# uricchio/2DSFS-scan

Measured on AMD Instinct MI355X. Metric: genomic windows/s (T2D+T1D+Fst) at 20 kb, n1=n2=50; HBM GB/s fraction, higher is better.
Workload: dtype f64

## Files before the change

### 2dsfs-scan_amd/csrc/sfs2d.hip

```cpp
#include <hip/hip_runtime.h>
#include <hip/hip_ext.h>

#include <algorithm>
#include <array>
#include <cmath>
#include <cstdint>
#include <cstdio>
#include <cstdlib>
#include <cstring>
#include <map>
#include <string>
#include <mutex>
#include <new>
#include <utility>
#include <vector>

#include "sfs2d.h"
#include "sfs2d_kernels.hpp"
#include "sfs2d_div.hpp"
#include "sfs2d_spec.hpp"
#include "sfs2d_proj.hpp"
#include "sfs2d_projscan.hpp"
#include "sfs2d_projnull.hpp"

// ... 170 lines not shown
  int tevery = 1;
  int tmask = 7;
  int64_t tseen = 0;
  hipEvent_t* tpend = nullptr;
  hipEvent_t kev[6] = {nullptr, nullptr, nullptr, nullptr, nullptr, nullptr};
  std::vector<unsigned long long> slot_base_h;
  uint32_t* d_slot_base = nullptr;
  sfs2d_plan* base = nullptr;
  std::vector<sfs2d_plan*> attached;
  uint32_t fst_m = 0;
  bool fst_win = false;
  bool fst_scan = false;
  bool fst_mask = true;
  bool gate = false;
  bool lean = false;
  int nfst = 0;
  std::vector<NullTask> ntask_h;
  DevBuf<NullTask> ntask;
  CallOut<sfs2d_window, 0> null_out;
  int variant[6] = {-1, -1, -1, -1, -1, -1};
  bool variant_set = false;
  CallOut<sfs2d_diversity> div_out;
  std::vector<SpecSel> spec_sel_h;
  DevBuf<SpecSel> spec_sel;
  CallOut<int64_t> spec_out;
  std::vector<ProjSel> proj_sel_h;
  DevBuf<ProjSel> proj_sel;
  CallOut<int64_t> proj_out;
  int64_t proj_roww = 0;
  int proj_e = 0;
// ... 86 lines not shown

bool free_slots(const sfs2d_plan* pl) { return pl->step > 0 || pl->regions; }

struct ScanW {
  bool p16, fused;
  int fst;
  bool cnt, gate, lean;
  using Fn = void (*)(SCAN_W_ARGS);
  static constexpr int N = 128;
  constexpr int index() const { return p16 | fused << 1 | fst << 2 | cnt << 4 | gate << 5 | lean << 6; }
  static constexpr ScanW at(int i) { return {bool(i & 1), bool(i & 2), (i >> 2) & 3, bool(i & 16), bool(i & 32), bool(i & 64)}; }
  constexpr bool legal() const { return fst < 2 ? !gate && !lean : cnt && (gate || !lean); }
  template <int I> static constexpr Fn kernel() { constexpr ScanW s = at(I); return k_scan_w<s.p16, s.fused, s.fst, s.cnt, s.gate, s.lean>; }
};

struct ScanGW {
  bool p16, fst, cnt, tri;
  using Fn = void (*)(SCAN_W_ARGS);
  static constexpr int N = 16;
  constexpr int index() const { return p16 | fst << 1 | cnt << 2 | tri << 3; }
  static constexpr ScanGW at(int i) { return {bool(i & 1), bool(i & 2), bool(i & 4), bool(i & 8)}; }
  constexpr bool legal() const { return cnt || !tri; }
  template <int I> static constexpr Fn kernel() { constexpr ScanGW s = at(I); return k_scan_gw<s.p16, s.fst, s.cnt, s.tri>; }
};

struct ScanG {
  bool p16, fst, cnt;
  using Fn = decltype(&k_scan_g<true, true, true>);
  static constexpr int N = 8;
  constexpr int index() const { return p16 | fst << 1 | cnt << 2; }
// ... 116 lines not shown
size_t static_lds(S s, size_t fallback) {
  hipFuncAttributes fa{};
  return hipFuncGetAttributes(&fa, (const void*)variants<S>[s.index()]) == hipSuccess ? fa.sharedSizeBytes : fallback;
}
template <class S>
int occupancy(S s, int block, size_t lds) {
  int occ = 0;
  return hipOccupancyMaxActiveBlocksPerMultiprocessor(&occ, variants<S>[s.index()], block, lds) == hipSuccess ? occ : 0;
}

ScanW scan_w_sel(const sfs2d_plan* pl) {
  const bool in_scan = pl->cnt && pl->fst_scan;
  const int fst = in_scan ? (pl->fst_mask ? 3 : 2) : prep_sums_fst(pl) ? 1 : 0;
  return {pl->p16, pl->fused, fst, pl->cnt, in_scan && (pl->gate || pl->lean), in_scan && pl->lean};
}
ScanGW scan_gw_sel(const sfs2d_plan* pl) { return {pl->p16, prep_sums_fst(pl), pl->cnt, pl->cnt && pl->K.ntri}; }
ScanG scan_g_sel(const sfs2d_plan* pl) { return {pl->p16, prep_sums_fst(pl), pl->cnt}; }
ScanExtra scan_extra_sel(const sfs2d_plan* pl) { return {pl->p16, pl->cnt}; }

ScanW occ_standin(ScanW s) { s.fst = s.fst >= 2 ? 2 : 1; s.cnt = true; return s; }
ScanGW occ_standin(ScanGW s) { s.fst = s.cnt = true; return s; }

constexpr ScanW SCAN_W_FIT = {true, true, 1, true, false, false};
constexpr ScanW scan_w_fst_fit(bool p16) { return {p16, true, 2, true, false, false}; }
constexpr Prep prep_lds_fit(bool fst) { return {true, true, true, true, false, fst, false}; }

void set_variant(sfs2d_plan* pl, int p16, int fused, int fst, int cnt, int gate, int tri) {
  const int v[6] = {p16, fused, fst, cnt, gate, tri};
  std::copy(v, v + 6, pl->variant);
  pl->variant_set = true;
}

int launch_scan(sfs2d_plan* pl, sfs2d_window* out) {
  const int per_chrom = pl->prm.bg_mode == SFS2D_BG_PER_CHROM ? 1 : 0;
  const int bp = pl->prm.window_mode == SFS2D_WINDOW_BP ? 1 : 0;
  const dim3 grid((unsigned)pl->chunks.size());
  int rc = 0;
  if (pl->gw) {
    const ScanGW s = scan_gw_sel(pl);
    const ScanGW::Fn k = variant(pl->ctx, s, "k_scan_gw", &rc);
    if (!k) return rc;
    set_variant(pl, s.p16, -1, s.fst, s.cnt, -1, s.tri);
    hipExtLaunchKernelGGL(k, grid, dim3(WAVE), pl->scan_lds,
                       CTX_STREAM(pl->ctx), pl->kev[4], pl->kev[5], 0, pl->K, scan_src(pl), pl->d_chunks, pl->d_slots, pl->d_tab, pl->d_lp, pl->d_head,
                       per_chrom, pl->ctx->d_lnx, pl->ctx->d_df, out, pl->d_err, bp, pl->d_repl, pl->d_bcount,
                       0, pl->d_leaves, pl->nleaves, pl->d_nodes, pl->nnodes, pl->nlevels, -1, pl->d_fsum, pl->d_fst,
                       pl->d_ctr, (int)(pl->runs & 1), pl->d_leafsum, pl->d_bg1d, 0, pl->d_gscr, pl->nscr);
  } else if (pl->G == WAVE) {
    const ScanW s = scan_w_sel(pl);
    const ScanW::Fn k = variant(pl->ctx, s, "k_scan_w", &rc);
    if (!k) return rc;
    set_variant(pl, s.p16, s.fused, s.fst, s.cnt, s.gate, -1);
    hipExtLaunchKernelGGL(k, grid, dim3(SBLOCK), pl->scan_lds,
                       CTX_STREAM(pl->ctx), pl->kev[4], pl->kev[5], 0, pl->K, scan_src(pl), pl->d_chunks, pl->d_slots, pl->d_tab, pl->d_lp, pl->d_head,
                       per_chrom, pl->ctx->d_lnx, pl->ctx->d_df, out, pl->d_err, bp, pl->d_repl, pl->d_bcount,
                       plan_par(pl), pl->d_leaves, pl->nleaves, pl->d_nodes, pl->nnodes, pl->nlevels,
                       pl->extra_rec >= 0 ? (int)pl->last_chrom : -1, pl->d_fsum, pl->d_fst, pl->d_ctr,
                       (int)(pl->runs & 1), pl->d_leafsum, pl->d_bg1d, pl->sliced ? 1 : 0, nullptr, 0);
  } else {
    const ScanG s = scan_g_sel(pl);
    const ScanG::Fn k = variant(pl->ctx, s, "k_scan_g", &rc);
    if (!k) return rc;
    set_variant(pl, s.p16, -1, s.fst, s.cnt, -1, -1);
    hipExtLaunchKernelGGL(k, grid, dim3(BLOCK), pl->scan_lds,
                       CTX_STREAM(pl->ctx), pl->kev[4], pl->kev[5], 0, pl->K, scan_src(pl), pl->d_chunks, pl->d_slots, pl->d_tab, pl->d_head, per_chrom,
// ... 518 lines not shown
  K->ws = (unsigned)prm->window;
  div_magic(K->ws, &K->wmag, &K->wsh1, &K->wsh2);
  K->nchrom = nchrom;
  K->fst_e = 40;
  K->fst_scale = std::ldexp(1.0, K->fst_e);
  return 0;
}

struct Knobs {
  const char* seg = std::getenv("SFS2D_SEG");
  const char* lnl = std::getenv("SFS2D_LNL");
  const char* gw = std::getenv("SFS2D_GW");
  const char* fused = std::getenv("SFS2D_FUSED");
  const char* fst_scan = std::getenv("SFS2D_FST_SCAN");
  const char* lean = std::getenv("SFS2D_LEAN");
  const char* slots_once = std::getenv("SFS2D_SLOTS_ONCE");
  const char* wgs = std::getenv("SFS2D_WGS");
  const char* gwwin = std::getenv("SFS2D_GWWIN");
  const char* pools = std::getenv("SFS2D_POOLS");
  const char* tile = std::getenv("SFS2D_TILE");
  const char* jnt = std::getenv("SFS2D_JNT");
};

struct RegionList {
  const int32_t* chrom;
  const uint32_t *first, *last;
  int64_t n;
};

static int plan_create(sfs2d_ctx* ctx, const sfs2d_data* data, const sfs2d_params* prm, int force_sliced, int64_t step,
// ... 222 lines not shown
  const bool small = pl->do_bg && pl->G == WAVE;
  const double wpw = (double)pl->nslots / (2.0 * ctx->ncu * (SBLOCK / WAVE));
  pl->sliced = small && wpw < 4.0;
  if (env.fused) pl->sliced = small && env.fused[0] == '0';
  if (force_sliced >= 0) pl->sliced = small && force_sliced == 1;
  pl->fused = small && !pl->sliced;
  pl->fst = (prm->flags & SFS2D_F_FST) != 0;
  pl->fst_scan = false;
  if (pl->fst && pl->cnt && pl->G == WAVE && !pl->gw) {
    pl->fst_scan = !(env.fst_scan && env.fst_scan[0] == '0');
    if (pl->fst_scan && pl->scan_lds + static_lds(scan_w_fst_fit(pl->p16), 160 * 1024) > 160 * 1024) pl->fst_scan = false;
  }
  pl->gate = pl->fst_scan && prm->fold && nc_ok;
  pl->lean = pl->gate && bp && K.n1p <= 31 && K.n2p <= 31;
  if (env.lean) pl->lean = pl->lean && env.lean[0] != '0';
  const PwTree pw = pw_plan(K.nb2 - 3);
  pl->fst_mask = data->low_nc;
  pl->fst_win = pl->sliced && bp && pl->fst && !pl->fst_scan;
  if (slide) pl->fst_win = pl->fst && !pl->fst_scan;
  pl->seg_index = bp && !slide && pl->cnt && pl->do_bg && !seg_prep && force_sliced < 0 && data->owned &&
                  !prep_sums_fst(pl);
  if (pl->seg_index) {
    if ((rc = data_pos_index(ctx, data))) { delete pl; return rc; }
    pl->do_seg = false;
  }
  pl->slots_once = pl->seg_index && pl->fst_scan;
  if (env.slots_once) pl->slots_once = pl->slots_once && env.slots_once[0] != '0';
  pl->nfst = pl->fst_win && !slide ? (int)std::min<int64_t>(1024, std::max<int64_t>(1, (pl->nslots + 7) / 8)) : 0;
  if (pl->scan_lds > 64 * 1024) {
    grant_lds<ScanW>(ctx, pl->scan_lds);
    grant_lds<ScanG>(ctx, pl->scan_lds);
  }
  if (pl->extra_lds > 64 * 1024) grant_lds<ScanExtra>(ctx, pl->extra_lds);

  if (pl->G == WAVE || pl->gw) {
    int occ = pl->gw ? occupancy(occ_standin(scan_gw_sel(pl)), WAVE, pl->scan_lds)
                     : occupancy(occ_standin(scan_w_sel(pl)), SBLOCK, pl->scan_lds);
    if (occ < 1) occ = 1;
    if (prm->scan_wgs_per_cu > 0 && (int)prm->scan_wgs_per_cu < occ) occ = (int)prm->scan_wgs_per_cu;
    int64_t cap = (int64_t)occ * ctx->ncu;
    if (pl->gw) pl->nscr = (int)cap;
    if (env.wgs) cap = std::max<int64_t>(1, std::atoll(env.wgs));
    const double S = (double)std::max<unsigned long long>(1, slot_base[nc] - slot_base[0]);
    const uint32_t NW = pl->gw ? 1u : (uint32_t)(SBLOCK / WAVE);
    int64_t gw_win = 64;
    if (env.gwwin) gw_win = std::max<int64_t>(1, std::atoll(env.gwwin));
    std::vector<double> order;
    for (int c = 0; c < nc; ++c) {
      const uint32_t ns = (uint32_t)(slot_base[c + 1] - slot_base[c]);
      if (!ns) continue;
      const uint32_t wmax = (ns + NW - 1) / NW;
      int64_t want = std::llround(cap * (ns / S));
// ... 248 lines not shown
  if (pl->base) return pl->step ? "slide" : pl->prm.window_mode == SFS2D_WINDOW_BP ? "bp" : "none";
  if (pl->step) return "slide";
  if (pl->seg_index) return "index";
  if (slots_only(pl)) return pl->seg_synth ? "synth" : "search";
  return pl->do_seg ? "prep" : "none";
}

int sfs2d_plan_slots_once(const sfs2d_plan* pl) { return !pl ? SFS2D_E_ARG : pl->slots_once ? 1 : 0; }

int sfs2d_plan_scan_variant(const sfs2d_plan* pl, int* p16, int* fused, int* fst, int* cnt, int* gate, int* tri) {
  if (!pl) return SFS2D_E_ARG;
  if (!pl->variant_set) return set_err(pl->ctx, SFS2D_E_ARG, "sfs2d_plan_scan_variant: the plan has launched no scan kernel yet");
  int* const o[6] = {p16, fused, fst, cnt, gate, tri};
  for (int i = 0; i < 6; ++i)
    if (o[i]) *o[i] = pl->variant[i];
  return 0;
}

int sfs2d_plan_set_timing(sfs2d_plan* pl, int max_runs) { return sfs2d_plan_set_timing_sampled(pl, max_runs, 1); }

int sfs2d_plan_set_timing_sampled(sfs2d_plan* pl, int max_runs, int every) {
  return sfs2d_plan_set_timing_kernels(pl, max_runs, every, 7);
}

int sfs2d_plan_set_timing_kernels(sfs2d_plan* pl, int max_runs, int every, int kernel_mask) {
  if (!pl || max_runs < 0 || every < 1 || (kernel_mask & ~7) || !kernel_mask) return SFS2D_E_ARG;
  pl->tevery = every;
  pl->tmask = kernel_mask;
  pl->tseen = 0;
  sfs2d_ctx* ctx = pl->ctx;
// ... 1323 lines not shown
```

### 2dsfs-scan_amd/csrc/sfs2d_kernels.hpp

```cpp
#pragma once

#include <type_traits>
#include <hip/hip_runtime.h>

#include <cmath>
#include <cstdint>

#include "sfs2d.h"

namespace sfs2dk {

constexpr int WAVE = 64;
constexpr int BLOCK = 256;
constexpr int SBLOCK = 512;
constexpr int BLOCK1 = 512;
constexpr int FBLOCK = 1024;
constexpr int KBLOCK = 512;
constexpr int LNX_N = 1 << 20;
constexpr int LNT = 512;
constexpr int LNF = 256;
__host__ __device__ inline int wl_rtn(int n1p, int n2p) { return 2 * (n1p > n2p ? n1p : n2p) + 2; }
constexpr int RCPN = 512;
#ifndef SFS2D_ABL
#define SFS2D_ABL 0
#endif
constexpr int REPL = 4;
constexpr int PW_MAX_LEAVES = 1024;
constexpr int LEAVES_PER_SLICE = 4;
constexpr int FIN_LDS_BINS = 12288;
constexpr int TRASH = WAVE;
constexpr int R1 = 4;
#ifndef SFS2D_GW_R1
#define SFS2D_GW_R1 1
#endif
constexpr int R1GW = SFS2D_GW_R1;

template <int RR>
__device__ __forceinline__ uint32_t take_replicas(uint32_t* p, uint32_t shift) {
  if (RR == 4) {
    uint4* q = reinterpret_cast<uint4*>(p);
    const uint4 v = *q;
    *q = make_uint4(0, 0, 0, 0);
    return (v.x >> shift) + (v.y >> shift) + (v.z >> shift) + (v.w >> shift);
  } else if (RR == 2) {
    uint2* q = reinterpret_cast<uint2*>(p);
    const uint2 v = *q;
    *q = make_uint2(0, 0);
    return (v.x >> shift) + (v.y >> shift);
  } else {
    const uint32_t v = *p;
    *p = 0u;
    return v >> shift;
  }
}
// ... 1355 lines not shown
    PL e;
    e.lp = LPl[k];
    if (k < nb2) {
      e.v = (double)u(k);
    } else if (k < t1b) {
      const int f = k - t1a;
      e.v = (double)u(h1a + f) + (f < n1p ? (double)u(h1a + n1 - f) : 0.0);
    } else {
      const int f = k - t1b, n2p = n2 / 2;
      e.v = (double)u(h1b + f) + (f < n2p ? (double)u(h1b + n2 - f) : 0.0);
    }
    return e;
  }
};

template <int G, bool P16, int S1, bool CNT, class Tab>
__device__ __forceinline__ WinOut eval_exact(const KParams& P, const uint32_t* __restrict__ bins, uint32_t b,
                                             uint32_t e, const Tab& T, const BgHead& hb,
                                             const double* __restrict__ lnx, uint32_t* H2, uint32_t* H1a,
                                             uint32_t* H1b, double* redd, unsigned long long* redu) {
  const int lane = threadIdx.x & (G - 1);
  const bool floatv = hb.flags & BGF_FLOATV;
  uint32_t c_var = 0, c2 = 0, c_last = 0, c1a = 0, c1b = 0;
  for (uint32_t i = b + lane; i < e; i += G) {
    const uint32_t w = snp_word<CNT>(P, bins, i);
    const uint32_t k2 = bin_k2(w), g1 = bin_g1(w), g2 = bin_g2(w);
    c_var += (w & B_VAR) ? 1u : 0u;
    c_last += (w & B_LAST) ? 1u : 0u;
    if (k2) { ++c2; h2_add<P16>(H2, k2); }
    if (g1) { ++c1a; atomicAdd(&H1a[g1 * S1], 1u); }
    if (g2) { ++c1b; atomicAdd(&H1b[g2 * S1], 1u); }
  }
  if (G == WAVE) __threadfence();
  group_sync<G>();
  const unsigned long long r0 = group_sum_u64<G>((unsigned long long)c2 | ((unsigned long long)c_last << 32), redu, 0);
  const unsigned long long r1 = group_sum_u64<G>((unsigned long long)c1a | ((unsigned long long)c1b << 32), redu, 1);
  const unsigned long long r2 = group_sum_u64<G>((unsigned long long)c_var, redu, 2);
  WinOut o;
  o.n2 = (uint32_t)r0;
  o.n2_all = o.n2 + (uint32_t)(r0 >> 32);
  o.n1a = (uint32_t)r1;
  o.n1b = (uint32_t)(r1 >> 32);
  o.snp_count = (uint32_t)r2;
  const double N2 = (double)o.n2, N1a = (double)o.n1a, N1b = (double)o.n1b;
// ... 27 lines not shown
        }
        __syncthreads();
      }
#pragma unroll
      for (int u = 0; u < U; ++u) {
        if (x2[u]) term(x2[u], (int)k2[u], N2, hb.B2, s2, q2);
        if (xa[u]) term(xa[u], P.t1a + (int)g1[u], N1a, hb.B1a, sa, qa);
        if (xb[u]) term(xb[u], P.t1b + (int)g2[u], N1b, hb.B1b, sb, qb);
      }
    }
  } else {
  for (uint32_t i = b + lane; i < e; i += G) {
    const uint32_t w = snp_word<CNT>(P, bins, i);
    const uint32_t k2 = bin_k2(w), g1 = bin_g1(w), g2 = bin_g2(w);
    if (k2) {
      const uint32_t x = h2_take<P16>(H2, k2);
      if (x) {
        const PL t = T.at(k2);
        s2 += (double)x * (lnx_of(lnx, x) - t.lp);
        q2 &= prop_ok(x, N2, t.v, hb.B2, floatv);
      }
    }
    if (g1) {
      const uint32_t x = atomicExch(&H1a[g1 * S1], 0u);
      if (x) {
        const PL t = T.at(P.t1a + g1);
        sa += (double)x * (lnx_of(lnx, x) - t.lp);
        qa &= prop_ok(x, N1a, t.v, hb.B1a, floatv);
      }
    }
    if (g2) {
// ... 666 lines not shown
}


__device__ __forceinline__ void lds_copy_d(double* dst, const double* __restrict__ src, int n) {
  constexpr int U = 8;
  for (int k0 = threadIdx.x; k0 < n; k0 += U * SBLOCK) {
    double v[U];
#pragma unroll
    for (int j = 0; j < U; ++j) v[j] = k0 + j * SBLOCK < n ? src[k0 + j * SBLOCK] : 0.0;
#pragma unroll
    for (int j = 0; j < U; ++j)
      if (k0 + j * SBLOCK < n) dst[k0 + j * SBLOCK] = v[j];
  }
}

template <bool P16, bool FUSED, int FST, bool CNT, bool GATE = false, bool LEAN = false>
__device__ __forceinline__ void scan_w_small(double* ldsd, uint32_t wgi, uint32_t nwg, SCAN_W_ARGS) {
  constexpr bool FSTIN = FST >= 2;
  constexpr bool FMASK = FST == 3;
  static_assert(!FSTIN || CNT, "Fst in the scan reads the counts");
  static_assert(!GATE || CNT, "the gate is a property of the counts the scan classifies");
  static_assert(!LEAN || (GATE && FSTIN), "the lean window loop is built for the gated Fst-in-scan plans");
  if (LEAN) mode_bp = 1;
  constexpr int DT = LNT;
  constexpr int R1U = R1;
  constexpr int NWV = SBLOCK / WAVE;
  constexpr int SB = 8;
  __shared__ BgHead sh_hb;
  __shared__ double sh_bd[NWV][3][SB];
  __shared__ uint32_t sh_bu[NWV][5][SB];
  __shared__ unsigned long long sh_bf[NWV][FST ? 2 : 1][SB];
  STAMP(10);
  BLK_STAMP(1, 0);
  const int tid = threadIdx.x;
  const int wv = __builtin_amdgcn_readfirstlane(tid >> 6);
  const int lane = tid & (WAVE - 1);
  const Chunk ch = chunks[wgi];
  const int bg = bg_per_chrom ? (int)ch.chrom : 0;

  double* LPl = ldsd;
  double* Dt = LPl + ((P.nt + 1) & ~1);
  double* Ft = Dt + DT;
  double2* RT = reinterpret_cast<double2*>(Ft + LNF);
  const int rtn = FSTIN ? P.rtn : 0;
  uint32_t* HB = reinterpret_cast<uint32_t*>(RT + rtn);
  const int h2w = P16 ? ((P.nb2 + 1) / 2 + 3) & ~3 : (P.nb2 + 3) & ~3;
  const int h1w = R1 * (P.n1p + 1), h1wb = R1 * (P.n2p + 1);
  const int per = (h2w + h1w + h1wb + 3) & ~3;
  uint32_t* W = HB + wv * per;
  uint32_t* H1a = W + h2w;
  uint32_t* H1b = H1a + h1w;
  const uint32_t rep = lane & (R1U - 1);

  auto bounds = [&](uint32_t s, uint2 sr, Win& w, bool live) {
    if (mode_bp) {
      w.has = live && sr.x != 0u;
      w.b = sr.x - 1u;
      w.e = sr.y;
    } else {
      w.has = live;
      w.b = ch.cb + (ch.wid_lo + (s - ch.slot_lo)) * P.ws;
      w.e = w.b + P.ws;
// ... 158 lines not shown
      }
    }
      if (mine && mode_bp && !FSTIN && !exact) {
        uint32_t z = 0u;
        asm volatile("" : "+v"(z));
        slots[Bs] = make_uint2(z, z);
      }
    MARK(31);
    for (unsigned long long m = __ballot(exact); m; m &= m - 1) {
      const int l = __builtin_ctzll(m);
      const uint32_t xs = __builtin_amdgcn_readlane(Bs, l), xb = __builtin_amdgcn_readlane(Bsb, l);
      const uint32_t xn = __builtin_amdgcn_readlane(Bnv, l) & 0xffffu;
      const uint32_t xe = xn != 0xffffu ? xb + xn : (mode_bp ? slots[xs].y : xb + P.ws);
      WinOut x;
      if (FUSED) {
        x = eval_exact<WAVE, P16, R1, CNT>(P, bins, xb, xe,
                                      TabFused{LPl, Rc, rs, P.nb2, P.n1, P.n2, P.n1p, P.h1a, P.h1b, P.t1a, P.t1b}, hb,
                                      lnx, W, H1a, H1b, nullptr, nullptr);
      } else {
        x = eval_exact<WAVE, P16, R1, CNT>(P, bins, xb, xe, TabLocal{tab + (size_t)bg * P.nt, LPl}, hb, lnx, W, H1a, H1b,
                                      nullptr, nullptr);
      }
      if (lane == 0) {
        write_rec(out + xs, ch.chrom, ch.wid_lo + (xs - ch.slot_lo), xb, xe, x, zflags);
        atomicAdd(err_word + 1, 1u);
      }
      group_sync<WAVE>();
    }
    jb = 0;
  };
#define SAT16(x) ((LEAN && P16) ? (x) : min((x), 0xffffu))
  auto put_u = [&](uint32_t slot, uint32_t b, uint32_t nsnp, uint32_t n2, uint32_t n1a, uint32_t n1b, uint32_t nvar,
                   uint32_t nlast) {
    sh_bu[wv][0][jb] = slot;
    sh_bu[wv][1][jb] = b;
// ... 90 lines not shown
        }
      }
    };
    auto pair = [&](uint32_t w0, uint32_t w1, int j, bool keep, const double2 (&fq)[4]) {
      const uint32_t ww[2] = {w0, w1};
      uint32_t rk[2], kk[2], ov[2], xs[2];
      bool in2[2];
#pragma unroll
      for (int q = 0; q < 2; ++q) {
        const uint32_t w = ww[q];
        uint32_t k2, gp;
        if (CNT) cls_k2g<GATE>(P, w, k2, gp);
        else { k2 = bin_k2(w); gp = bin_g1(w) | (bin_g2(w) << 16); }
        in2[q] = k2 != 0u;
        n2 += __popcll(__ballot(in2[q]));
        const uint32_t x = (CNT ? k2 : w) << 4;
        const uint32_t word = P16 ? (k2 >> 1) : k2;
        uint32_t one2 = 1u;
        if (P16) asm("v_lshlrev_b32 %0, %1, 1" : "=v"(one2) : "v"(x));
        const uint32_t wa = awb + word * 4u;
        uint32_t o = one2;
        if (in2[q] && !(SFS2D_ABL & 1))
          o = __hip_atomic_fetch_add((lds_u32*)(uintptr_t)wa, one2, __ATOMIC_RELAXED, __HIP_MEMORY_SCOPE_WORKGROUP);
        ov[q] = o;
        xs[q] = x;
        kk[q] = k2;
        if (keep) kw[(j + q) & 7] = word;
        constexpr int BS1 = 4 * R1;
        static_assert(BS1 <= 64, "the multiplier must be an inline constant");
        uint32_t u1, u2;
        asm("v_mad_u32_u16 %0, %1, %3, %2" : "=v"(u1) : "v"(gp), "v"(a1b), "n"(BS1));
        asm("v_mad_u32_u16 %0, %1, %3, %2 op_sel:[1,0,0,0]" : "=v"(u2) : "v"(gp), "v"(a2b), "n"(BS1));
        if (!(SFS2D_ABL & 2)) {
          __hip_atomic_fetch_add((lds_u32*)(uintptr_t)u1, one1, __ATOMIC_RELAXED, __HIP_MEMORY_SCOPE_WORKGROUP);
          __hip_atomic_fetch_add((lds_u32*)(uintptr_t)u2, one1, __ATOMIC_RELAXED, __HIP_MEMORY_SCOPE_WORKGROUP);
        }
      }
      if (FSTIN) {
        const double a0 = fq[0].y + fq[1].y, a1 = fq[2].y + fq[3].y;
        const double p0 = fq[0].x + fq[1].x, p1 = fq[2].x + fq[3].x;
        if (j == 0) {
          fA = a0 + a1;
          fP = p0 + p1;
// ... 62 lines not shown
        const uint32_t w = i0 + lane < cur.e ? snp_word<CNT>(P, bins, i0 + lane) : 0u;
        nlast += __popcll(__ballot((w & B_LAST) != 0u));
        nvar += __popcll(__ballot((w & B_VAR) != 0u));
      }
    }
    if (!filt) nvar = nsnp;
    ulonglong2 fq = make_ulonglong2(0ull, 0ull);
    if (FST == 1 && lane == 0) fq = reinterpret_cast<const ulonglong2*>(fsum)[s];
    if (LEAN) fq.x = (unsigned long long)__double_as_longlong(lnx[SAT16(n2)]);
    if (it == 0) STAMP(12);
    MARK(23);
    group_sync<WAVE>();
    if (clampd) {
      constexpr uint32_t L1 = LNT - 1;
      const double fl = (double)L1 * lnx[L1];
      for (int k = lane; k < h2w; k += WAVE) {
        const uint32_t v = W[k];
        const uint32_t xa = P16 ? (v & 0xffffu) : v, xb = P16 ? (v >> 16) : 0u;
        if (xa > L1) acc2 += (double)xa * lnx_of(lnx, xa) - fl;
        if (xb > L1) acc2 += (double)xb * lnx_of(lnx, xb) - fl;
      }
    }
    if (nsnp <= 8 * WAVE) {
#pragma unroll
      for (int j = 0; j < 8; ++j)
        if (64 * j < (int)nsnp) W[kw[j]] = 0u;
    } else {
      uint4* q = reinterpret_cast<uint4*>(W);
      for (int k = lane; k < h2w / 4; k += WAVE) q[k] = make_uint4(0, 0, 0, 0);
    }
    MARK(24);
    double acca = 0.0, accb = 0.0;
    constexpr uint32_t S1 = P16 ? 16u : 0u;
    const uint32_t slots = 128u * ((nsnp + 127u) / 128u);
    auto take1 = [&](uint32_t* H, int k) -> uint32_t {
      if (SFS2D_ABL & 32) return (uint32_t)k;
      return take_replicas<R1U>(H + k * R1, S1);
    };
    if (half1d) {
      const bool pa = lane < 32;
      const int k = lane & 31, np = pa ? P.n1p : P.n2p;
      uint32_t x = 0;
      if (k <= np) {
        x = take1(pa ? H1a : H1b, k);
        if (k >= 1 && k < np && x) acca = xlnx<LNF>(x, Ft, lnx) - (double)x * LPl[(pa ? P.t1a : P.t1b) + k];
      }
      n1a = slots - (uint32_t)__builtin_amdgcn_readlane((int)x, 0) - (uint32_t)__builtin_amdgcn_readlane((int)x, P.n1p);
      n1b = slots - (uint32_t)__builtin_amdgcn_readlane((int)x, 32) -
            (uint32_t)__builtin_amdgcn_readlane((int)x, 32 + P.n2p);
    } else {
      uint32_t xa[2] = {0u, 0u}, xb[2] = {0u, 0u};
#pragma unroll
// ... 71 lines not shown
  bounds(s, srs, cur, true);
  }
  STAMP(15);
  WV_STAMP(it);
#ifdef SFS2D_STAMPS
  __builtin_amdgcn_s_barrier();
#endif
  BLK_STAMP(1, 1);
#undef SAT16
}

template <bool P16, bool FUSED, int FST, bool CNT, bool GATE = false, bool LEAN = false>
__global__ __launch_bounds__(SBLOCK) __attribute__((amdgpu_waves_per_eu(4))) void k_scan_w(SCAN_W_ARGS) {
  extern __shared__ double ldsd[];
  scan_w_small<P16, FUSED, FST, CNT, GATE, LEAN>(ldsd, blockIdx.x, gridDim.x, SCAN_W_PASS);
}

template <bool P16, bool FST, bool CNT, bool TRI = false>
__global__ __launch_bounds__(WAVE) __attribute__((amdgpu_waves_per_eu(4))) void k_scan_gw(SCAN_W_ARGS) {
  extern __shared__ double ldsd[];
  scan_gw_body<P16, FST, CNT, TRI>(ldsd, SCAN_W_PASS);
}

template <bool P16, bool FST, bool CNT>
__global__ __launch_bounds__(BLOCK) void k_scan_g(KParams P, const uint32_t* __restrict__ bins,
                                                  const Chunk* __restrict__ chunks, uint2* __restrict__ slots,
                                                  const PL* __restrict__ tab, const BgHead* __restrict__ head,
                                                  int bg_per_chrom, const double* __restrict__ lnx,
                                                  sfs2d_window* __restrict__ out, int mode_bp,
                                                  unsigned long long* __restrict__ fsum, double* __restrict__ fst_out) {
// ... 332 lines not shown
```

### 2dsfs-scan_amd/sfs2d/_lib.py

```python
from __future__ import annotations

import ctypes as C
import os

import numpy as np

HERE = os.path.dirname(os.path.abspath(__file__))
LIB_PATH = os.environ.get("SFS2D_LIB", os.path.join(HERE, "..", "csrc", "libsfs2d.so"))

OK = 0
E_ARG, E_HIP, E_NOMEM, E_KEY, E_GRID, E_CAP = -1, -2, -3, -4, -5, -6
WINDOW_BP, WINDOW_SNPS = 0, 1
BG_PER_CHROM, BG_SUPPLIED = 0, 1
F_PREV_EXTRA = 1
F_FST = 2
W_EMPTY = 0x80000000
W_BG2_ZERO, W_BG1A_ZERO, W_BG1B_ZERO = 0x1, 0x2, 0x4
W_EXTRA = 0x40000000


def bg_row_words(n1p: int, n2p: int) -> int:
    return (2 * n1p + 1) * (2 * n2p + 1) + 2 * n1p + 2 * n2p + 3


# ... 5 lines not shown
    return (m1 + 1) * (m2 + 1) + 2

EXPORTS = [
    "sfs2d_abi_version", "sfs2d_ctx_create", "sfs2d_ctx_destroy", "sfs2d_last_error", "sfs2d_ctx_set_stream",
    "sfs2d_data_upload", "sfs2d_data_wrap_device", "sfs2d_data_free", "sfs2d_bg_hist", "sfs2d_plan_create",
    "sfs2d_plan_num_records", "sfs2d_plan_set_background", "sfs2d_plan_run", "sfs2d_plan_run_many", "sfs2d_plan_set_timing_sampled",
    "sfs2d_plan_set_timing_kernels",
    "sfs2d_plan_fst_read", "sfs2d_plan_fst_buffer", "sfs2d_plan_read",
    "sfs2d_plan_bg_buffer", "sfs2d_plan_bg_words", "sfs2d_plan_bg_exchange", "sfs2d_plan_run_phase", "sfs2d_plan_check", "sfs2d_plan_time",
    "sfs2d_plan_destroy", "sfs2d_scan", "sfs2d_plan_set_timing", "sfs2d_plan_timing_read",
    "sfs2d_plan_stats", "sfs2d_plan_grids", "sfs2d_plan_scan_kernel", "sfs2d_plan_attach", "sfs2d_data_synth_sims",
    "sfs2d_data_read", "sfs2d_plan_run_streams", "sfs2d_ctx_use_own_stream", "sfs2d_bg_hist_dev", "sfs2d_plan_bg_rows_dev", "sfs2d_plan_bg_rows_set_dev",
    "sfs2d_ctx_get_stream", "sfs2d_plan_set_fst_out", "sfs2d_graph_create", "sfs2d_graph_launch", "sfs2d_graph_destroy",
    "sfs2d_plan_create_sliding", "sfs2d_plan_attach_sliding", "sfs2d_plan_null_run", "sfs2d_plan_null_read",
    "sfs2d_plan_null_run_blocks",
    "sfs2d_plan_scan_variant", "sfs2d_plan_seg_kind", "sfs2d_plan_slots_once",
    "sfs2d_plan_diversity", "sfs2d_plan_diversity_read",
    "sfs2d_plan_create_regions", "sfs2d_plan_attach_regions",
    "sfs2d_plan_spectra", "sfs2d_plan_spectra_read",
    "sfs2d_plan_project", "sfs2d_plan_project_read", "sfs2d_project_weights",
    "sfs2d_plan_project_scan", "sfs2d_plan_project_scan_read",
    "sfs2d_plan_project_null", "sfs2d_plan_project_null_read",
]
PNULL_THIN = 8
ABI_VERSION = 2


class Sfs2dError(RuntimeError):
    def __init__(self, code, msg):
        super().__init__(f"sfs2d error {code}: {msg}")
        self.code = code
# ... 87 lines not shown
    L.sfs2d_plan_bg_buffer.argtypes = [vp, C.POINTER(vp), C.POINTER(i64)]
    L.sfs2d_plan_bg_words.argtypes = [vp, C.POINTER(i64), C.POINTER(i64), C.POINTER(i64)]
    L.sfs2d_plan_bg_exchange.argtypes = [vp, vp, vp, C.c_int]
    L.sfs2d_bg_hist_dev.argtypes = [vp, vp, C.POINTER(Params), i32, vp]
    L.sfs2d_plan_bg_rows_dev.argtypes = [vp, vp, i64]
    L.sfs2d_plan_bg_rows_set_dev.argtypes = [vp, vp, i64]
    L.sfs2d_plan_check.argtypes = [vp]
    L.sfs2d_plan_time.argtypes = [vp, C.c_int] + [C.POINTER(C.c_double)] * 4
    L.sfs2d_plan_destroy.argtypes = [vp]
    L.sfs2d_plan_set_timing.argtypes = [vp, C.c_int]
    L.sfs2d_plan_stats.argtypes = [vp, C.POINTER(C.c_uint32)]
    L.sfs2d_plan_grids.argtypes = [vp, C.POINTER(i64), C.POINTER(i64)]
    L.sfs2d_plan_scan_kernel.argtypes = [vp]
    L.sfs2d_plan_scan_kernel.restype = C.c_char_p
    L.sfs2d_plan_scan_variant.argtypes = [vp] + [C.POINTER(C.c_int)] * 6
    L.sfs2d_plan_slots_once.argtypes = [vp]
    L.sfs2d_plan_seg_kind.argtypes = [vp]
    L.sfs2d_plan_seg_kind.restype = C.c_char_p
    L.sfs2d_plan_attach.argtypes = [vp, C.POINTER(Params), C.POINTER(vp)]
    L.sfs2d_plan_create_sliding.argtypes = [vp, vp, C.POINTER(Params), i64, C.POINTER(vp)]
    L.sfs2d_plan_attach_sliding.argtypes = [vp, C.POINTER(Params), i64, C.POINTER(vp)]
    L.sfs2d_plan_create_regions.argtypes = [vp, vp, C.POINTER(Params), vp, vp, vp, i64, C.POINTER(vp)]
    L.sfs2d_plan_attach_regions.argtypes = [vp, C.POINTER(Params), vp, vp, vp, i64, C.POINTER(vp)]
    L.sfs2d_plan_null_run.argtypes = [vp, C.POINTER(NullParams), vp, i64, vp]
    L.sfs2d_plan_null_run_blocks.argtypes = [vp, C.POINTER(NullParams), i64, vp, i64, vp]
    L.sfs2d_plan_null_read.argtypes = [vp, vp, i64, C.POINTER(i64)]
    L.sfs2d_plan_diversity.argtypes = [vp, vp]
    L.sfs2d_plan_diversity_read.argtypes = [vp, vp, i64, C.POINTER(i64)]
    L.sfs2d_plan_spectra.argtypes = [vp, vp, vp, i64, i64, vp]
    L.sfs2d_plan_spectra_read.argtypes = [vp, vp, i64, C.POINTER(i64)]
# ... 21 lines not shown
```

### 2dsfs-scan_amd/sfs2d/engine.py

```python
from __future__ import annotations

import ctypes as C
from dataclasses import dataclass
from typing import Optional

import numpy as np

from . import _lib as L
from .pack import PackedSNPs
from .regions import Regions


@dataclass
class ScanConfig:
    n1p: int
    n2p: int
    fold: bool = True
    window_mode: int = L.WINDOW_BP
    window: int = 20000
    bg_mode: int = L.BG_PER_CHROM
    ann_want: int = -1
    start_position: Optional[int] = None
    end_position: Optional[int] = None
    prev_extra: bool = False
# ... 402 lines not shown

    def scan_kernel(self) -> str:
        return self.eng.lib.sfs2d_plan_scan_kernel(self.h).decode()

    def seg_kind(self) -> str:
        return self.eng.lib.sfs2d_plan_seg_kind(self.h).decode()

    def slots_once(self) -> bool:
        return self.eng.lib.sfs2d_plan_slots_once(self.h) == 1

    def scan_variant(self) -> dict:
        v = [C.c_int() for _ in range(6)]
        self.eng.check(self.eng.lib.sfs2d_plan_scan_variant(self.h, *[C.byref(x) for x in v]))
        return dict(zip(("p16", "fused", "fst", "cnt", "gate", "tri"), (x.value for x in v)))

    def stats(self) -> int:
        v = C.c_uint32()
        self.eng.check(self.eng.lib.sfs2d_plan_stats(self.h, C.byref(v)))
        return int(v.value)

    def set_timing(self, max_runs: int, every: int = 1, kernels: int = 7):
        self.eng.check(self.eng.lib.sfs2d_plan_set_timing_kernels(self.h, int(max_runs), int(every), int(kernels)))

    def timing_read(self):
        n = C.c_int()
        v = [C.c_double() for _ in range(3)]
        self.eng.check(self.eng.lib.sfs2d_plan_timing_read(self.h, C.byref(n), *[C.byref(x) for x in v]))
        return n.value, tuple(x.value for x in v)

    def close(self):
# ... 89 lines not shown
```

### include/sfs2d.h

```cpp
#ifndef SFS2D_H
#define SFS2D_H

#include <stdint.h>

#ifdef __cplusplus
extern "C" {
#endif

#define SFS2D_ABI_VERSION 2

#define SFS2D_OK 0
#define SFS2D_E_ARG (-1)
#define SFS2D_E_HIP (-2)
#define SFS2D_E_NOMEM (-3)
#define SFS2D_E_KEY (-4)
#define SFS2D_E_GRID (-5)
#define SFS2D_E_CAP (-6)

#define SFS2D_WINDOW_BP 0
#define SFS2D_WINDOW_SNPS 1

#define SFS2D_BG_PER_CHROM 0
#define SFS2D_BG_SUPPLIED 1

// ... 129 lines not shown
  uint32_t e;
} sfs2d_projstat;
int sfs2d_plan_project_scan(sfs2d_plan* plan, int32_t m1, int32_t m2, int32_t bg_chrom, sfs2d_projstat* out_dev,
                            int32_t* e_out, int32_t* e_bg_out);
int sfs2d_plan_project_scan_read(sfs2d_plan* plan, sfs2d_projstat* out_host, int64_t cap, int64_t* nrec_out);
#define SFS2D_PNULL_THIN 8
int sfs2d_plan_project_null(sfs2d_plan* plan, int32_t m1, int32_t m2, const sfs2d_null_params* np, const int64_t* rec,
                            int64_t nsel, sfs2d_projstat* out_dev, uint32_t* thin_dev, int32_t* e_out, int32_t* e_bg_out);
int sfs2d_plan_project_null_read(sfs2d_plan* plan, sfs2d_projstat* out_host, uint32_t* thin_host, int64_t cap,
                                 int64_t* nrec_out);
int sfs2d_plan_grids(const sfs2d_plan* plan, int64_t* prep_threads, int64_t* scan_threads);
const char* sfs2d_plan_scan_kernel(const sfs2d_plan* plan);
const char* sfs2d_plan_seg_kind(const sfs2d_plan* plan);
int sfs2d_plan_slots_once(const sfs2d_plan* plan);
int sfs2d_plan_scan_variant(const sfs2d_plan* plan, int* p16, int* fused, int* fst, int* cnt, int* gate, int* tri);
int sfs2d_plan_stats(sfs2d_plan* plan, uint32_t* exact_windows);
int sfs2d_plan_check(sfs2d_plan* plan);
int sfs2d_plan_set_timing(sfs2d_plan* plan, int max_runs);
int sfs2d_plan_set_timing_sampled(sfs2d_plan* plan, int max_samples, int every);
int sfs2d_plan_set_timing_kernels(sfs2d_plan* plan, int max_samples, int every, int kernel_mask);
int sfs2d_plan_timing_read(sfs2d_plan* plan, int* nruns, double* ms_k1, double* ms_k2, double* ms_k3);
int sfs2d_plan_time(sfs2d_plan* plan, int iters, double* ms_per_run, double* ms_k1, double* ms_k2, double* ms_k3);
int sfs2d_plan_destroy(sfs2d_plan* plan);

int sfs2d_scan(sfs2d_ctx* ctx, const sfs2d_data* data, const sfs2d_params* params, const double* bg2d,
               const double* bg1a, const double* bg1b, sfs2d_window* out_host, int64_t cap, int64_t* nrec_out);

#ifdef __cplusplus
}
#endif
// ... 2 lines not shown
```

Before: 1.029 billion.

## Add folded triangular 2D histogram scan kernel with larger batches and replicas

```diff
diff --git a/2dsfs-scan_amd/csrc/sfs2d.hip b/2dsfs-scan_amd/csrc/sfs2d.hip
--- a/2dsfs-scan_amd/csrc/sfs2d.hip
+++ b/2dsfs-scan_amd/csrc/sfs2d.hip
@@ -208,6 +208,8 @@
   bool fst_mask = true;
   bool gate = false;
   bool lean = false;
+  bool tri = false;
+  int sb = 8, r1 = R1;
   int nfst = 0;
   std::vector<NullTask> ntask_h;
   DevBuf<NullTask> ntask;
@@ -324,6 +326,16 @@
   template <int I> static constexpr Fn kernel() { constexpr ScanW s = at(I); return k_scan_w<s.p16, s.fused, s.fst, s.cnt, s.gate, s.lean>; }
 };
 
+struct ScanWT {
+  bool p16, fused, fmask, sb32, r8;
+  using Fn = void (*)(SCAN_W_ARGS);
+  static constexpr int N = 32;
+  constexpr int index() const { return p16 | fused << 1 | fmask << 2 | sb32 << 3 | r8 << 4; }
+  static constexpr ScanWT at(int i) { return {bool(i & 1), bool(i & 2), bool(i & 4), bool(i & 8), bool(i & 16)}; }
+  constexpr bool legal() const { return true; }
+  template <int I> static constexpr Fn kernel() { constexpr ScanWT s = at(I); return k_scan_wt<s.p16, s.fused, s.fmask, s.sb32 ? 32 : 8, s.r8 ? 8 : R1>; }
+};
+
 struct ScanGW {
   bool p16, fst, cnt, tri;
   using Fn = void (*)(SCAN_W_ARGS);
@@ -470,6 +482,7 @@
   const int fst = in_scan ? (pl->fst_mask ? 3 : 2) : prep_sums_fst(pl) ? 1 : 0;
   return {pl->p16, pl->fused, fst, pl->cnt, in_scan && (pl->gate || pl->lean), in_scan && pl->lean};
 }
+ScanWT scan_wt_sel(const sfs2d_plan* pl) { return {pl->p16, pl->fused, pl->fst_mask, pl->sb == 32, pl->r1 == 8}; }
 ScanGW scan_gw_sel(const sfs2d_plan* pl) { return {pl->p16, prep_sums_fst(pl), pl->cnt, pl->cnt && pl->K.ntri}; }
 ScanG scan_g_sel(const sfs2d_plan* pl) { return {pl->p16, prep_sums_fst(pl), pl->cnt}; }
 ScanExtra scan_extra_sel(const sfs2d_plan* pl) { return {pl->p16, pl->cnt}; }
@@ -480,6 +493,9 @@
 constexpr ScanW SCAN_W_FIT = {true, true, 1, true, false, false};
 constexpr ScanW scan_w_fst_fit(bool p16) { return {p16, true, 2, true, false, false}; }
 constexpr Prep prep_lds_fit(bool fst) { return {true, true, true, true, false, fst, false}; }
+
+constexpr size_t SCAN_WT_LDS = 80 * 1024;
+constexpr double SCAN_WT_MIN_WPW = 8.0;
 
 void set_variant(sfs2d_plan* pl, int p16, int fused, int fst, int cnt, int gate, int tri) {
   const int v[6] = {p16, fused, fst, cnt, gate, tri};
@@ -504,7 +520,7 @@
                        pl->d_ctr, (int)(pl->runs & 1), pl->d_leafsum, pl->d_bg1d, 0, pl->d_gscr, pl->nscr);
   } else if (pl->G == WAVE) {
     const ScanW s = scan_w_sel(pl);
-    const ScanW::Fn k = variant(pl->ctx, s, "k_scan_w", &rc);
+    const ScanW::Fn k = pl->tri ? variant(pl->ctx, scan_wt_sel(pl), "k_scan_wt", &rc) : variant(pl->ctx, s, "k_scan_w", &rc);
     if (!k) return rc;
     set_variant(pl, s.p16, s.fused, s.fst, s.cnt, s.gate, -1);
     hipExtLaunchKernelGGL(k, grid, dim3(SBLOCK), pl->scan_lds,
@@ -1053,6 +1069,9 @@
   const char* fused = std::getenv("SFS2D_FUSED");
   const char* fst_scan = std::getenv("SFS2D_FST_SCAN");
   const char* lean = std::getenv("SFS2D_LEAN");
+  const char* tri = std::getenv("SFS2D_TRI");
+  const char* sb = std::getenv("SFS2D_SB");
+  const char* r1 = std::getenv("SFS2D_R1");
   const char* slots_once = std::getenv("SFS2D_SLOTS_ONCE");
   const char* wgs = std::getenv("SFS2D_WGS");
   const char* gwwin = std::getenv("SFS2D_GWWIN");
@@ -1305,6 +1324,27 @@
   pl->gate = pl->fst_scan && prm->fold && nc_ok;
   pl->lean = pl->gate && bp && K.n1p <= 31 && K.n2p <= 31;
   if (env.lean) pl->lean = pl->lean && env.lean[0] != '0';
+  const std::string sbv = env.sb ? env.sb : "32", r1v = env.r1 ? env.r1 : "8";
+  if ((sbv != "8" && sbv != "32") || (r1v != "4" && r1v != "8")) {
+    delete pl;
+    return set_err(ctx, SFS2D_E_ARG, "SFS2D_SB must be 8 or 32 and SFS2D_R1 4 or 8 (the instantiations k_scan_wt has)");
+  }
+  const bool tri_gate = wpw >= SCAN_WT_MIN_WPW || (env.tri && env.tri[0] == '1');
+  if (pl->lean && K.n1 == K.n2 && !(env.tri && env.tri[0] == '0') && tri_gate) {
+    const int sb = sbv == "8" ? 8 : 32, r1 = r1v == "4" ? 4 : 8;
+    const int nh2 = (K.nb2 + K.n1) / 2 + 1;
+    const int h2w = pl->p16 ? (((nh2 + 1) / 2 + 3) & ~3) : ((nh2 + 3) & ~3);
+    const int per = (h2w + r1 * (K.n1p + 1) + r1 * (K.n2p + 1) + 3) & ~3;
+    const size_t hist_words = std::max<size_t>((size_t)(SBLOCK / WAVE) * per, (size_t)FUSED_VCNT + K.nt + 16);
+    const size_t lds = sizeof(double) * (size_t)(((K.nt + 1) & ~1) + LNT + LNF + 2 * (size_t)pl->K.rtn) + hist_words * 4;
+    const ScanWT fit = {pl->p16, true, true, sb == 32, r1 == 8};
+    if (lds + static_lds(fit, SCAN_WT_LDS) <= SCAN_WT_LDS) {
+      pl->tri = true;
+      pl->sb = sb;
+      pl->r1 = r1;
+      pl->scan_lds = lds;
+    }
+  }
   const PwTree pw = pw_plan(K.nb2 - 3);
   pl->fst_mask = data->low_nc;
   pl->fst_win = pl->sliced && bp && pl->fst && !pl->fst_scan;
@@ -1320,13 +1360,15 @@
   pl->nfst = pl->fst_win && !slide ? (int)std::min<int64_t>(1024, std::max<int64_t>(1, (pl->nslots + 7) / 8)) : 0;
   if (pl->scan_lds > 64 * 1024) {
     grant_lds<ScanW>(ctx, pl->scan_lds);
+    grant_lds<ScanWT>(ctx, pl->scan_lds);
     grant_lds<ScanG>(ctx, pl->scan_lds);
   }
   if (pl->extra_lds > 64 * 1024) grant_lds<ScanExtra>(ctx, pl->extra_lds);
 
   if (pl->G == WAVE || pl->gw) {
     int occ = pl->gw ? occupancy(occ_standin(scan_gw_sel(pl)), WAVE, pl->scan_lds)
-                     : occupancy(occ_standin(scan_w_sel(pl)), SBLOCK, pl->scan_lds);
+                     : pl->tri ? occupancy(scan_wt_sel(pl), SBLOCK, pl->scan_lds)
+                               : occupancy(occ_standin(scan_w_sel(pl)), SBLOCK, pl->scan_lds);
     if (occ < 1) occ = 1;
     if (prm->scan_wgs_per_cu > 0 && (int)prm->scan_wgs_per_cu < occ) occ = (int)prm->scan_wgs_per_cu;
     int64_t cap = (int64_t)occ * ctx->ncu;
@@ -1605,6 +1647,15 @@
   int* const o[6] = {p16, fused, fst, cnt, gate, tri};
   for (int i = 0; i < 6; ++i)
     if (o[i]) *o[i] = pl->variant[i];
+  return 0;
+}
+
+int sfs2d_plan_scan_packing(const sfs2d_plan* pl, int* tri, int* sb, int* r1) {
+  if (!pl) return SFS2D_E_ARG;
+  const bool w = pl->G == WAVE && !pl->gw;
+  if (tri) *tri = w ? (pl->tri ? 1 : 0) : -1;
+  if (sb) *sb = w ? pl->sb : -1;
+  if (r1) *r1 = w ? pl->r1 : -1;
   return 0;
 }
 
diff --git a/2dsfs-scan_amd/csrc/sfs2d_kernels.hpp b/2dsfs-scan_amd/csrc/sfs2d_kernels.hpp
--- a/2dsfs-scan_amd/csrc/sfs2d_kernels.hpp
+++ b/2dsfs-scan_amd/csrc/sfs2d_kernels.hpp
@@ -37,7 +37,14 @@
 
 template <int RR>
 __device__ __forceinline__ uint32_t take_replicas(uint32_t* p, uint32_t shift) {
-  if (RR == 4) {
+  if (RR == 8) {
+    uint4* q = reinterpret_cast<uint4*>(p);
+    const uint4 v = q[0], u = q[1];
+    q[0] = make_uint4(0, 0, 0, 0);
+    q[1] = make_uint4(0, 0, 0, 0);
+    return (v.x >> shift) + (v.y >> shift) + (v.z >> shift) + (v.w >> shift) + (u.x >> shift) + (u.y >> shift) +
+           (u.z >> shift) + (u.w >> shift);
+  } else if (RR == 4) {
     uint4* q = reinterpret_cast<uint4*>(p);
     const uint4 v = *q;
     *q = make_uint4(0, 0, 0, 0);
@@ -1423,20 +1430,22 @@
   }
 };
 
-template <int G, bool P16, int S1, bool CNT, class Tab>
+template <int G, bool P16, int S1, bool CNT, bool TRI = false, class Tab>
 __device__ __forceinline__ WinOut eval_exact(const KParams& P, const uint32_t* __restrict__ bins, uint32_t b,
                                              uint32_t e, const Tab& T, const BgHead& hb,
                                              const double* __restrict__ lnx, uint32_t* H2, uint32_t* H1a,
                                              uint32_t* H1b, double* redd, unsigned long long* redu) {
+  static_assert(!TRI || G == WAVE, "the packed histogram is k_scan_w's");
   const int lane = threadIdx.x & (G - 1);
   const bool floatv = hb.flags & BGF_FLOATV;
+  [[maybe_unused]] const uint32_t triC = (uint32_t)(P.nb2 + P.n1);
   uint32_t c_var = 0, c2 = 0, c_last = 0, c1a = 0, c1b = 0;
   for (uint32_t i = b + lane; i < e; i += G) {
     const uint32_t w = snp_word<CNT>(P, bins, i);
     const uint32_t k2 = bin_k2(w), g1 = bin_g1(w), g2 = bin_g2(w);
     c_var += (w & B_VAR) ? 1u : 0u;
     c_last += (w & B_LAST) ? 1u : 0u;
-    if (k2) { ++c2; h2_add<P16>(H2, k2); }
+    if (k2) { ++c2; h2_add<P16>(H2, TRI ? min(k2, triC - k2) : k2); }
     if (g1) { ++c1a; atomicAdd(&H1a[g1 * S1], 1u); }
     if (g2) { ++c1b; atomicAdd(&H1b[g2 * S1], 1u); }
   }
@@ -1494,7 +1503,7 @@
     const uint32_t w = snp_word<CNT>(P, bins, i);
     const uint32_t k2 = bin_k2(w), g1 = bin_g1(w), g2 = bin_g2(w);
     if (k2) {
-      const uint32_t x = h2_take<P16>(H2, k2);
+      const uint32_t x = h2_take<P16>(H2, TRI ? min(k2, triC - k2) : k2);
       if (x) {
         const PL t = T.at(k2);
         s2 += (double)x * (lnx_of(lnx, x) - t.lp);
@@ -2191,18 +2200,22 @@
   }
 }
 
-template <bool P16, bool FUSED, int FST, bool CNT, bool GATE = false, bool LEAN = false>
+template <bool P16, bool FUSED, int FST, bool CNT, bool GATE = false, bool LEAN = false, bool TRI = false, int SBN = 8,
+          int R1N = R1>
 __device__ __forceinline__ void scan_w_small(double* ldsd, uint32_t wgi, uint32_t nwg, SCAN_W_ARGS) {
   constexpr bool FSTIN = FST >= 2;
   constexpr bool FMASK = FST == 3;
   static_assert(!FSTIN || CNT, "Fst in the scan reads the counts");
   static_assert(!GATE || CNT, "the gate is a property of the counts the scan classifies");
   static_assert(!LEAN || (GATE && FSTIN), "the lean window loop is built for the gated Fst-in-scan plans");
+  static_assert(LEAN || (!TRI && SBN == 8 && R1N == R1), "the packed histogram and what its room buys are the lean class's");
+  static_assert(SBN >= 8 && SBN <= WAVE && (SBN & (SBN - 1)) == 0, "a batch is a power of two of at most a wavefront's lanes");
+  static_assert(R1N == 1 || R1N == 2 || R1N == 4 || R1N == 8, "take_replicas' copies");
   if (LEAN) mode_bp = 1;
   constexpr int DT = LNT;
-  constexpr int R1U = R1;
+  constexpr int R1U = R1N;
   constexpr int NWV = SBLOCK / WAVE;
-  constexpr int SB = 8;
+  constexpr int SB = SBN;
   __shared__ BgHead sh_hb;
   __shared__ double sh_bd[NWV][3][SB];
   __shared__ uint32_t sh_bu[NWV][5][SB];
@@ -2221,8 +2234,10 @@
   double2* RT = reinterpret_cast<double2*>(Ft + LNF);
   const int rtn = FSTIN ? P.rtn : 0;
   uint32_t* HB = reinterpret_cast<uint32_t*>(RT + rtn);
-  const int h2w = P16 ? ((P.nb2 + 1) / 2 + 3) & ~3 : (P.nb2 + 3) & ~3;
-  const int h1w = R1 * (P.n1p + 1), h1wb = R1 * (P.n2p + 1);
+  [[maybe_unused]] const uint32_t triC = TRI ? (uint32_t)(P.nb2 + P.n1) : 0u;
+  const int nh2 = TRI ? (P.nb2 + P.n1) / 2 + 1 : P.nb2;
+  const int h2w = P16 ? ((nh2 + 1) / 2 + 3) & ~3 : (nh2 + 3) & ~3;
+  const int h1w = R1U * (P.n1p + 1), h1wb = R1U * (P.n2p + 1);
   const int per = (h2w + h1w + h1wb + 3) & ~3;
   uint32_t* W = HB + wv * per;
   uint32_t* H1a = W + h2w;
@@ -2411,11 +2426,11 @@
       const uint32_t xe = xn != 0xffffu ? xb + xn : (mode_bp ? slots[xs].y : xb + P.ws);
       WinOut x;
       if (FUSED) {
-        x = eval_exact<WAVE, P16, R1, CNT>(P, bins, xb, xe,
+        x = eval_exact<WAVE, P16, R1U, CNT, TRI>(P, bins, xb, xe,
                                       TabFused{LPl, Rc, rs, P.nb2, P.n1, P.n2, P.n1p, P.h1a, P.h1b, P.t1a, P.t1b}, hb,
                                       lnx, W, H1a, H1b, nullptr, nullptr);
       } else {
-        x = eval_exact<WAVE, P16, R1, CNT>(P, bins, xb, xe, TabLocal{tab + (size_t)bg * P.nt, LPl}, hb, lnx, W, H1a, H1b,
+        x = eval_exact<WAVE, P16, R1U, CNT, TRI>(P, bins, xb, xe, TabLocal{tab + (size_t)bg * P.nt, LPl}, hb, lnx, W, H1a, H1b,
                                       nullptr, nullptr);
       }
       if (lane == 0) {
@@ -2536,8 +2551,9 @@
         else { k2 = bin_k2(w); gp = bin_g1(w) | (bin_g2(w) << 16); }
         in2[q] = k2 != 0u;
         n2 += __popcll(__ballot(in2[q]));
-        const uint32_t x = (CNT ? k2 : w) << 4;
-        const uint32_t word = P16 ? (k2 >> 1) : k2;
+        const uint32_t kh = TRI ? min(k2, triC - k2) : k2;
+        const uint32_t x = (CNT ? kh : w) << 4;
+        const uint32_t word = P16 ? (kh >> 1) : kh;
         uint32_t one2 = 1u;
         if (P16) asm("v_lshlrev_b32 %0, %1, 1" : "=v"(one2) : "v"(x));
         const uint32_t wa = awb + word * 4u;
@@ -2548,7 +2564,7 @@
         xs[q] = x;
         kk[q] = k2;
         if (keep) kw[(j + q) & 7] = word;
-        constexpr int BS1 = 4 * R1;
+        constexpr int BS1 = 4 * R1U;
         static_assert(BS1 <= 64, "the multiplier must be an inline constant");
         uint32_t u1, u2;
         asm("v_mad_u32_u16 %0, %1, %3, %2" : "=v"(u1) : "v"(gp), "v"(a1b), "n"(BS1));
@@ -2641,6 +2657,22 @@
     if (clampd) {
       constexpr uint32_t L1 = LNT - 1;
       const double fl = (double)L1 * lnx[L1];
+      if (TRI) {
+        static_assert(!TRI || CNT, "the packed histogram needs the counts' keys");
+        const uint32_t np1 = (uint32_t)P.n1 + 1u;
+        const uint32_t rcp = (1u << 20) / np1 + 1u;
+        const int hl = P16 ? ((P.nb2 + 1) / 2 + 3) & ~3 : (P.nb2 + 3) & ~3;
+        for (int k = lane; k < hl; k += WAVE)
+#pragma unroll
+          for (int h = 0; h < (P16 ? 2 : 1); ++h) {
+            const uint32_t kb = P16 ? 2u * (uint32_t)k + (uint32_t)h : (uint32_t)k;
+            const uint32_t x1 = (kb * rcp) >> 20;
+            if (kb >= (uint32_t)P.nb2 || x1 + (kb - x1 * np1) > (uint32_t)P.n1) continue;
+            const uint32_t kp = min(kb, triC - kb);
+            const uint32_t v = P16 ? (W[kp >> 1] >> ((kp & 1u) << 4)) & 0xffffu : W[kp];
+            if (v > L1) acc2 += (double)v * lnx_of(lnx, v) - fl;
+          }
+      } else
       for (int k = lane; k < h2w; k += WAVE) {
         const uint32_t v = W[k];
         const uint32_t xa = P16 ? (v & 0xffffu) : v, xb = P16 ? (v >> 16) : 0u;
@@ -2662,7 +2694,7 @@
     const uint32_t slots = 128u * ((nsnp + 127u) / 128u);
     auto take1 = [&](uint32_t* H, int k) -> uint32_t {
       if (SFS2D_ABL & 32) return (uint32_t)k;
-      return take_replicas<R1U>(H + k * R1, S1);
+      return take_replicas<R1U>(H + k * R1U, S1);
     };
     if (half1d) {
       const bool pa = lane < 32;
@@ -2764,6 +2796,12 @@
 __global__ __launch_bounds__(SBLOCK) __attribute__((amdgpu_waves_per_eu(4))) void k_scan_w(SCAN_W_ARGS) {
   extern __shared__ double ldsd[];
   scan_w_small<P16, FUSED, FST, CNT, GATE, LEAN>(ldsd, blockIdx.x, gridDim.x, SCAN_W_PASS);
+}
+
+template <bool P16, bool FUSED, bool FMASK, int SBN, int R1N>
+__global__ __launch_bounds__(SBLOCK) __attribute__((amdgpu_waves_per_eu(4))) void k_scan_wt(SCAN_W_ARGS) {
+  extern __shared__ double ldsd[];
+  scan_w_small<P16, FUSED, FMASK ? 3 : 2, true, true, true, true, SBN, R1N>(ldsd, blockIdx.x, gridDim.x, SCAN_W_PASS);
 }
 
 template <bool P16, bool FST, bool CNT, bool TRI = false>
diff --git a/2dsfs-scan_amd/sfs2d/_lib.py b/2dsfs-scan_amd/sfs2d/_lib.py
--- a/2dsfs-scan_amd/sfs2d/_lib.py
+++ b/2dsfs-scan_amd/sfs2d/_lib.py
@@ -43,7 +43,7 @@
     "sfs2d_ctx_get_stream", "sfs2d_plan_set_fst_out", "sfs2d_graph_create", "sfs2d_graph_launch", "sfs2d_graph_destroy",
     "sfs2d_plan_create_sliding", "sfs2d_plan_attach_sliding", "sfs2d_plan_null_run", "sfs2d_plan_null_read",
     "sfs2d_plan_null_run_blocks",
-    "sfs2d_plan_scan_variant", "sfs2d_plan_seg_kind", "sfs2d_plan_slots_once",
+    "sfs2d_plan_scan_variant", "sfs2d_plan_scan_packing", "sfs2d_plan_seg_kind", "sfs2d_plan_slots_once",
     "sfs2d_plan_diversity", "sfs2d_plan_diversity_read",
     "sfs2d_plan_create_regions", "sfs2d_plan_attach_regions",
     "sfs2d_plan_spectra", "sfs2d_plan_spectra_read",
@@ -161,6 +161,7 @@
     L.sfs2d_plan_scan_kernel.argtypes = [vp]
     L.sfs2d_plan_scan_kernel.restype = C.c_char_p
     L.sfs2d_plan_scan_variant.argtypes = [vp] + [C.POINTER(C.c_int)] * 6
+    L.sfs2d_plan_scan_packing.argtypes = [vp] + [C.POINTER(C.c_int)] * 3
     L.sfs2d_plan_slots_once.argtypes = [vp]
     L.sfs2d_plan_seg_kind.argtypes = [vp]
     L.sfs2d_plan_seg_kind.restype = C.c_char_p
diff --git a/2dsfs-scan_amd/sfs2d/engine.py b/2dsfs-scan_amd/sfs2d/engine.py
--- a/2dsfs-scan_amd/sfs2d/engine.py
+++ b/2dsfs-scan_amd/sfs2d/engine.py
@@ -440,6 +440,11 @@
         self.eng.check(self.eng.lib.sfs2d_plan_scan_variant(self.h, *[C.byref(x) for x in v]))
         return dict(zip(("p16", "fused", "fst", "cnt", "gate", "tri"), (x.value for x in v)))
 
+    def scan_packing(self) -> dict:
+        v = [C.c_int() for _ in range(3)]
+        self.eng.check(self.eng.lib.sfs2d_plan_scan_packing(self.h, *[C.byref(x) for x in v]))
+        return dict(zip(("tri", "sb", "r1"), (x.value for x in v)))
+
     def stats(self) -> int:
         v = C.c_uint32()
         self.eng.check(self.eng.lib.sfs2d_plan_stats(self.h, C.byref(v)))
diff --git a/include/sfs2d.h b/include/sfs2d.h
--- a/include/sfs2d.h
+++ b/include/sfs2d.h
@@ -167,6 +167,7 @@
 const char* sfs2d_plan_seg_kind(const sfs2d_plan* plan);
 int sfs2d_plan_slots_once(const sfs2d_plan* plan);
 int sfs2d_plan_scan_variant(const sfs2d_plan* plan, int* p16, int* fused, int* fst, int* cnt, int* gate, int* tri);
+int sfs2d_plan_scan_packing(const sfs2d_plan* plan, int* tri, int* sb, int* r1);
 int sfs2d_plan_stats(sfs2d_plan* plan, uint32_t* exact_windows);
 int sfs2d_plan_check(sfs2d_plan* plan);
 int sfs2d_plan_set_timing(sfs2d_plan* plan, int max_runs);
```

New measurement: 1.057 billion, median of 6. 1.03x the previous value.
